# rehakvoj1/BIH-GPU-Raytracer

Hardware: NVIDIA B200
Metric: Mrays/s (higher is better)
Workload: dtype f32

## Files before the change

### bih-gpu-raytracer_b200/csrc/trace.cu

```cuda
#include "bihrt_internal.cuh"
#include <float.h>

#define FULL 0xffffffffu
#define NONE 0xFFFFFFFFu
#define TRACE_THREADS 128
#define TRACE_MIN_BLOCKS 8
constexpr int NODE_STEPS = 4;

#define OCT_MIXED 8
#define BOX_EPS 2.384185791015625e-07f

#define DET_EPS __uint_as_float(0x358637beu)

struct Hit { float t; int slot; };

__device__ __forceinline__ float fmin3(float a, float b, float c) { float r; asm("min.f32 %0, %1, %2, %3;" : "=f"(r) : "f"(a), "f"(b), "f"(c)); return r; }
__device__ __forceinline__ float fmax3(float a, float b, float c) { float r; asm("max.f32 %0, %1, %2, %3;" : "=f"(r) : "f"(a), "f"(b), "f"(c)); return r; }

__device__ __forceinline__ uint32_t pack_colour(uint32_t hits, int samples) {
    const float fh = (float)hits, fm = (float)(samples - (int)hits), fs = (float)samples;
    float cr = __fdiv_rn(__fadd_rn(__fmul_rn(fh, 255.f), __fmul_rn(fm, 20.f)), fs);
    float cb = __fdiv_rn(__fmul_rn(fm, 40.f), fs);
    cr = fmaxf(0.f, fminf(255.f, cr));
    cb = fmaxf(0.f, fminf(255.f, cb));
    return ((uint32_t)(int)cb << 16) | ((uint32_t)(int)cr << 8) | (uint32_t)(int)cr;
}

__device__ __forceinline__ float mt_det(float dx, float dy, float dz, float e1x, float e1y, float e1z, float e2x, float e2y, float e2z,
                                        float& px, float& py, float& pz) {
    px = __fsub_rn(__fmul_rn(dy, e2z), __fmul_rn(e2y, dz));
    py = __fsub_rn(__fmul_rn(dz, e2x), __fmul_rn(e2z, dx));
    pz = __fsub_rn(__fmul_rn(dx, e2y), __fmul_rn(e2x, dy));
    return __fadd_rn(__fadd_rn(__fmul_rn(e1x, px), __fmul_rn(e1y, py)), __fmul_rn(e1z, pz));
}
__device__ __forceinline__ float mt_u(float ox, float oy, float oz, const float4& q0, float px, float py, float pz, float inv,
                                      float& tx, float& ty, float& tz) {
    tx = __fsub_rn(ox, q0.x); ty = __fsub_rn(oy, q0.y); tz = __fsub_rn(oz, q0.z);
    return __fmul_rn(__fadd_rn(__fadd_rn(__fmul_rn(tx, px), __fmul_rn(ty, py)), __fmul_rn(tz, pz)), inv);
}
__device__ __forceinline__ float mt_v(float dx, float dy, float dz, float e1x, float e1y, float e1z, float tx, float ty, float tz, float inv,
                                      float& qx, float& qy, float& qz) {
    qx = __fsub_rn(__fmul_rn(ty, e1z), __fmul_rn(e1y, tz));
    qy = __fsub_rn(__fmul_rn(tz, e1x), __fmul_rn(e1z, tx));
    qz = __fsub_rn(__fmul_rn(tx, e1y), __fmul_rn(e1x, ty));
    return __fmul_rn(__fadd_rn(__fadd_rn(__fmul_rn(dx, qx), __fmul_rn(dy, qy)), __fmul_rn(dz, qz)), inv);
}

template <bool COUNTED, bool FIRST, bool RANGE = false, bool TWO_SIDED = false>
__device__ __forceinline__ void test_leaf(const char* __restrict__ first_tri, float ox, float oy, float oz,
                                          float dx, float dy, float dz, Hit& h, uint32_t& ntris, uint32_t& wleaf,
                                          const float* tlo_p = nullptr) {
    const float4* p = reinterpret_cast<const float4*>(first_tri);
    for (;;) {
        const float4 q0 = __ldg(p), q1 = __ldg(p + 1), q2 = __ldg(p + 2);
        if (COUNTED) { ntris++; const uint32_t am = __activemask(); wleaf += ((threadIdx.x & 31) == __ffs(am) - 1); }
        const float e1x = q0.w, e1y = q1.x, e1z = q1.y, e2x = q1.z, e2y = q1.w, e2z = q2.x;
        float px, py, pz;
        const float det = mt_det(dx, dy, dz, e1x, e1y, e1z, e2x, e2y, e2z, px, py, pz);
        if (!((TWO_SIDED ? fabsf(det) : det) < DET_EPS)) {
            const float inv = __frcp_rn(det);
            float tx, ty, tz;
            const float u = mt_u(ox, oy, oz, q0, px, py, pz, inv, tx, ty, tz);
            if (!(u < 0.f || u > 1.f)) {
                float qx, qy, qz;
                const float v = mt_v(dx, dy, dz, e1x, e1y, e1z, tx, ty, tz, inv, qx, qy, qz);
                if (!(v < 0.f || __fadd_rn(u, v) > 1.f)) {
                    const float t = __fmul_rn(__fadd_rn(__fadd_rn(__fmul_rn(e2x, qx), __fmul_rn(e2y, qy)), __fmul_rn(e2z, qz)), inv);
                    if (t > (RANGE ? *tlo_p : 0.f) && t < h.t) {
                        h.t = t; h.slot = (int)__float_as_uint(q2.w);
                        if (FIRST) break;
                    }
                }
            }
        }
        if (__float_as_uint(q2.z) & 1u) break;
        p += 3;
    }
}

template <int MODE, bool COUNTED, bool Q>
__global__ void __launch_bounds__(TRACE_THREADS, TRACE_MIN_BLOCKS) k_trace(TraceArgs a) {
    constexpr int STACK_DEPTH = Q ? STACK_DEPTH_QUALITY : STACK_DEPTH_PARITY;
    constexpr bool COVER = MODE == 1;
    constexpr bool OCTS = MODE == 1;
    constexpr bool LIST = MODE == 0 || MODE == 3 || MODE == 4;
    constexpr bool RANGE = MODE == 3 || MODE == 4;
    constexpr bool TWO_SIDED = MODE == 4;
    __shared__ __align__(16) float s_ray[TRACE_THREADS * 10];
    const int lane = threadIdx.x & 31;
    const uint32_t lt = (1u << lane) - 1u;
    float* my_ray = s_ray + threadIdx.x * 10;
    const char* __restrict__ nodes_b = reinterpret_cast<const char*>(a.nodes);
    const char* __restrict__ tris_b = reinterpret_cast<const char*>(a.tris);
    const BihTri* __restrict__ tris = a.tris;
    const uint32_t nu = a.hdr->nu;
    if (a.hdr->status != 0) return;
    if ((a.hdr->quality != 0) != Q) {
        if (blockIdx.x == 0 && threadIdx.x == 0 && a.status_map) *a.status_map = 0x100u;
        return;
    }
    const float blo[3] = { a.hdr->lo[0], a.hdr->lo[1], a.hdr->lo[2] }, bhi[3] = { a.hdr->hi[0], a.hdr->hi[1], a.hdr->hi[2] };
    uint32_t nnodes = 0, ntris = 0, maxsp = 0;
    uint32_t wnode = 0, wleaf = 0;

    uint64_t total;
    int tx = 1;
    if (LIST) total = a.tile_cost ? (((uint64_t)a.nrays + 1023u) >> 10) << 10 : (uint64_t)a.nrays;
    else {
        tx = (a.w + 31) / 32;
        const int ty = (a.h + 31) / 32, T = tx * ty;
        const int my_tiles = T > a.shard_index ? (T - a.shard_index + a.shard_count - 1) / a.shard_count : 0;
        total = ((uint64_t)my_tiles * 1024u) << a.gshift;
    }
    const int gshift = LIST ? 0 : a.gshift;
    const int nsamp = LIST ? 1 : ((a.s_end - a.s_begin) >> gshift);
    uint32_t my_queue = 0;
    if (a.queues > 1) { asm("mov.u32 %0, %%smid;" : "=r"(my_queue)); my_queue %= (uint32_t)a.queues; }
    uint64_t pool_next = 0, pool_end = 0;
    long long unit_t0 = 0; uint32_t unit_tile = 0xFFFFFFFFu;
    bool exhausted = false;

    uint64_t item = ~0ull;
    int s = 0, s0 = 0;
    uint32_t hits = 0, pixel = 0, pxy = 0;
    float ix = 1.f, iy = 1.f, iz = 1.f, nx = 0.f, ny = 0.f, nz = 0.f, bpad = 0.f;
    uint32_t cur = NONE;
    float rMin = 0.f, pMin = 0.f, pMax = 0.f;
    Hit h; h.t = FLT_MAX; h.slot = -1;
    bool tracing = false;
    uint4 stack[STACK_DEPTH];
    int sp = 0;
#define STACK_RESET() do { sp = 0; } while (0)
#define STACK_PUSH(item) do { stack[sp] = (item); sp++; } while (0)
#define STACK_POP(e) do { sp--; (e) = stack[sp]; } while (0)
    const uint32_t root_ref = BIH_REF_NODE(0, a.hdr->root_axis);
    const bool direct = MODE == 1 && gshift > 0 && !(a.flags & BIHRT_RENDER_COUNTS);
    const uint32_t ray_smem = (uint32_t)__cvta_generic_to_shared(my_ray);

    for (;;) {
        const uint32_t busy = ~__ballot_sync(FULL, cur == NONE);
        if (busy == 0) {
            bool want_item = false, finishing = false;
            if (cur == NONE) {
                if (tracing) {
                    tracing = false;
                    if (MODE == 1) hits += (h.slot >= 0);
                    else if (RANGE) {
                        const bool hit = h.slot >= 0;
                        const bool rec = a.out_u || a.out_v || a.out_ng;
                        float u = 0.f, v = 0.f, gx = 0.f, gy = 0.f, gz = 0.f;
                        int32_t prim = -1;
                        if (hit && (rec || a.out_prim)) {
                            const float4* tq = reinterpret_cast<const float4*>(tris + h.slot);
                            const float4 q0 = __ldg(tq), q1 = __ldg(tq + 1), q2 = __ldg(tq + 2);
                            prim = (int32_t)__float_as_uint(q2.y);
                            if (rec) {
                                const float e1x = q0.w, e1y = q1.x, e1z = q1.y, e2x = q1.z, e2y = q1.w, e2z = q2.x;
                                const float2 dxy = *reinterpret_cast<const float2*>(my_ray + 6);
                                const float dx = dxy.x, dy = dxy.y, dz = my_ray[8];
                                float px, py, pz, tx, ty, tz, qx, qy, qz;
                                const float inv = __frcp_rn(mt_det(dx, dy, dz, e1x, e1y, e1z, e2x, e2y, e2z, px, py, pz));
                                u = mt_u(my_ray[0], my_ray[2], my_ray[4], q0, px, py, pz, inv, tx, ty, tz);
                                v = mt_v(dx, dy, dz, e1x, e1y, e1z, tx, ty, tz, inv, qx, qy, qz);
                                gx = __fsub_rn(__fmul_rn(e1y, e2z), __fmul_rn(e1z, e2y));
                                gy = __fsub_rn(__fmul_rn(e1z, e2x), __fmul_rn(e1x, e2z));
                                gz = __fsub_rn(__fmul_rn(e1x, e2y), __fmul_rn(e1y, e2x));
                            }
                        }
                        if (a.out_t) a.out_t[item] = hit ? h.t : FLT_MAX;
                        if (a.out_slot) a.out_slot[item] = h.slot;
                        if (a.out_prim) a.out_prim[item] = prim;
                        if (a.out_u) a.out_u[item] = u;
                        if (a.out_v) a.out_v[item] = v;
                        if (a.out_ng) { float* g = a.out_ng + 3 * item; g[0] = gx; g[1] = gy; g[2] = gz; }
                    } else {
                        const uint64_t o = MODE == 0 ? item : (uint64_t)pixel * (uint32_t)a.spp + (uint32_t)(s0 + s);
                        if (a.out_t) a.out_t[o] = h.t;
                        if (a.out_slot) a.out_slot[o] = h.slot;
                        if (a.out_prim) a.out_prim[o] = h.slot >= 0 ? (int32_t)tris[h.slot].prim : -1;
                    }
                    s++;
                    if (s == nsamp) {
                        if (MODE == 1 && gshift > 0) finishing = true;
                        else if (MODE == 1 && (a.flags & BIHRT_RENDER_COUNTS)) a.fb[pixel] = hits;
                        else if (MODE == 1) a.fb[pixel] = pack_colour(hits, nsamp);
                        item = ~0ull;
                    }
                }
                want_item = (item == ~0ull);
            }
            if (MODE == 1 && gshift > 0) {
                const uint32_t fin = __ballot_sync(FULL, finishing);
                if (finishing) {
                    const uint32_t same = __match_any_sync(fin, pixel);
                    const uint32_t sum = __reduce_add_sync(same, hits);
                    if (lane == __ffs(same) - 1) {
                        if (direct) a.fb[pixel] = pack_colour(sum, nsamp << gshift);
                        else if (sum) atomicAdd(&a.fb[pixel], sum);
                    }
                }
            }
            if (!LIST && a.tile_cost && unit_tile != 0xFFFFFFFFu) {
                if (lane == 0) atomicMax(a.tile_cost + unit_tile, (uint32_t)min((unsigned long long)(clock64() - unit_t0) >> 8, 0xFFFFFFFFull));
                unit_tile = 0xFFFFFFFFu;
            }
            uint32_t want = __ballot_sync(FULL, want_item);
            while (want && !exhausted) {
                if (pool_next >= pool_end) {
                    uint64_t base = ~0ull;
                    uint32_t got = 0;
                    if (lane == 0) {
                        const uint32_t ilc = (uint32_t)a.il_count, ili = (uint32_t)a.il_index, ics = (uint32_t)a.il_cshift;
                        if (a.queues <= 1) {
                            const uint64_t fetched = atomicAdd(a.work, 32u); got = 32;
                            const uint64_t lu = fetched >> 5;
                            base = ilc > 1 ? ((((lu >> ics) * ilc + ili) << ics) | (lu & ((1u << ics) - 1u))) << 5 : fetched;
                            if (base >= total) base = ~0ull;
                        } else {
                            const uint32_t tshift = 10 + gshift, ushift = 5 + gshift;
                            const uint64_t ntile = (total + ((1ull << tshift) - 1)) >> tshift;
                            for (uint32_t k = 0; k < (uint32_t)a.queues; k++) {
                                uint32_t q = my_queue + k; if (q >= (uint32_t)a.queues) q -= (uint32_t)a.queues;
                                if (q >= ntile) continue;
                                const uint32_t upt = (1u << ushift) / ilc;
                                const uint64_t units = ((ntile - q + a.queues - 1) / a.queues) * upt;
                                if (ld_relaxed(a.work + q) >= units) continue;
                                const uint32_t u = atomicAdd(a.work + q, 1u);
                                if (u >= units) continue;
                                const uint32_t lu = u % upt;
                                const uint64_t b = (((uint64_t)(u / upt) * a.queues + q) << tshift) + ((uint64_t)((((lu >> ics) * ilc + ili) << ics) | (lu & ((1u << ics) - 1u))) << 5);
                                if (b < total) { base = b; got = 32; break; }
                            }
                        }
                    }
                    base = __shfl_sync(FULL, base, 0);
                    got = __shfl_sync(FULL, got, 0);
                    if (LIST && a.tile_cost && unit_tile != 0xFFFFFFFFu) {
                        if (lane == 0) atomicMax(a.tile_cost + unit_tile, (uint32_t)min((unsigned long long)(clock64() - unit_t0) >> 8, 0xFFFFFFFFull));
                        unit_tile = 0xFFFFFFFFu;
                    }
                    if (base == ~0ull) { exhausted = true; break; }
                    pool_next = base;
                    pool_end = min(base + got, total);
                    if (a.tile_cost && unit_tile == 0xFFFFFFFFu) {
                        const uint32_t m = (uint32_t)(base >> (10 + gshift));
                        unit_tile = a.tile_order ? __ldg(a.tile_order + m) : m;
                        unit_t0 = clock64();
                    }
                }
                const uint64_t avail = pool_end - pool_next;
                const uint32_t rank = __popc(want & lt);
                const bool served = want_item && (uint64_t)rank < avail;
                if (served) {
                    item = pool_next + rank; s = 0; hits = 0; want_item = false;
                    if (LIST && a.tile_cost) {
                        const uint32_t mi = (uint32_t)(item >> 10);
                        const uint64_t ray = ((uint64_t)(a.tile_order ? __ldg(a.tile_order + mi) : mi) << 10) | (item & 1023u);
                        item = ray < (uint64_t)a.nrays ? ray : ~0ull;
                        if (item == ~0ull) want_item = true;
                    }
                    if (MODE == 0 && a.perm && item != ~0ull) item = __ldg(a.perm + item);
                    if (!LIST) {
                        const uint64_t pix = item >> gshift;
                        s0 = a.s_begin + (int)((uint32_t)item & ((1u << gshift) - 1u)) * nsamp;
                        const uint32_t mi = (uint32_t)(pix >> 10), q = (uint32_t)pix & 1023u;
                        const uint32_t m = a.tile_order ? __ldg(a.tile_order + mi) : mi;
                        const int tile = a.shard_index + (int)m * a.shard_count;
                        const int px = (tile % tx) * 32 + (int)((q >> 5) & 3u) * 8 + (int)(q & 7u);
                        const int py = (tile / tx) * 32 + (int)(q >> 7) * 4 + (int)((q >> 3) & 3u);
                        if (px < a.w && py < a.h) { pixel = (uint32_t)(py * a.w + px); pxy = (uint32_t)px | ((uint32_t)py << 16); }
                        else item = ~0ull;
                        if (item == ~0ull) want_item = true;
                    }
                }
                pool_next += min((uint64_t)__popc(want), avail);
                want = __ballot_sync(FULL, want_item);
            }
            if (cur == NONE && item != ~0ull) {
                float ox, oy, oz, dx, dy, dz;
                float tlo = 0.f, thi = FLT_MAX;
                bool live = true;
                if (RANGE) {
                    const float4* p = reinterpret_cast<const float4*>(a.rays_iv + item);
                    const float4 r0 = __ldg(p), r1 = __ldg(p + 1);
                    ox = r0.x; oy = r0.y; oz = r0.z; dx = r1.x; dy = r1.y; dz = r1.z;
                    tlo = fmaxf(r0.w, 0.f);
                    live = r0.w == r0.w && tlo < r1.w;
                    thi = fminf(r1.w, FLT_MAX);
                } else if (MODE == 0) {
                    const float* p = reinterpret_cast<const float*>(a.rays + item);
                    ox = __ldg(p); oy = __ldg(p + 1); oz = __ldg(p + 2); dx = __ldg(p + 3); dy = __ldg(p + 4); dz = __ldg(p + 5);
                } else {
                    const int px = (int)(pxy & 0xFFFFu), py = (int)(pxy >> 16);
                    const float ru = (a.flags & BIHRT_RENDER_JITTER) ? bihrt_jitter(a.seed, pixel, (uint32_t)(s0 + s), 0) : 0.5f;
                    const float rv = (a.flags & BIHRT_RENDER_JITTER) ? bihrt_jitter(a.seed, pixel, (uint32_t)(s0 + s), 1) : 0.5f;
                    const float uu = __fdiv_rn(__fadd_rn((float)px, ru), (float)a.w);
                    const float vv = __fdiv_rn(__fadd_rn((float)py, rv), (float)a.h);
                    ox = a.cam.origin[0]; oy = a.cam.origin[1]; oz = a.cam.origin[2];
                    dx = __fsub_rn(__fadd_rn(__fadd_rn(a.cam.lower_left[0], __fmul_rn(uu, a.cam.horizontal[0])), __fmul_rn(vv, a.cam.vertical[0])), ox);
                    dy = __fsub_rn(__fadd_rn(__fadd_rn(a.cam.lower_left[1], __fmul_rn(uu, a.cam.horizontal[1])), __fmul_rn(vv, a.cam.vertical[1])), oy);
                    dz = __fsub_rn(__fadd_rn(__fadd_rn(a.cam.lower_left[2], __fmul_rn(uu, a.cam.horizontal[2])), __fmul_rn(vv, a.cam.vertical[2])), oz);
                }
                ix = __frcp_rn(dx); iy = __frcp_rn(dy); iz = __frcp_rn(dz);
                nx = -__fmul_rn(ox, ix); ny = -__fmul_rn(oy, iy); nz = -__fmul_rn(oz, iz);
                bpad = __fmul_rn(BOX_EPS, fmaxf(fmaxf(fabsf(nx) <= FLT_MAX ? fabsf(nx) : 0.f, fabsf(ny) <= FLT_MAX ? fabsf(ny) : 0.f),
                                                fabsf(nz) <= FLT_MAX ? fabsf(nz) : 0.f));
                *reinterpret_cast<float2*>(my_ray) = make_float2(ox, ix); *reinterpret_cast<float2*>(my_ray + 2) = make_float2(oy, iy);
                *reinterpret_cast<float2*>(my_ray + 4) = make_float2(oz, iz); *reinterpret_cast<float2*>(my_ray + 6) = make_float2(dx, dy);
                my_ray[8] = dz;
                if (RANGE) my_ray[9] = tlo;
                h.t = RANGE ? thi : (MODE == 0 && a.any_hit) ? a.tmax : FLT_MAX; h.slot = -1; STACK_RESET(); tracing = true;
                bool in = nu > 0 && live;
                float tMin = __fmul_rn(__fsub_rn(ix < 0.f ? bhi[0] : blo[0], ox), ix);
                float tMax = __fmul_rn(__fsub_rn(ix < 0.f ? blo[0] : bhi[0], ox), ix);
                const float tymin = __fmul_rn(__fsub_rn(iy < 0.f ? bhi[1] : blo[1], oy), iy);
                const float tymax = __fmul_rn(__fsub_rn(iy < 0.f ? blo[1] : bhi[1], oy), iy);
                if ((tMin > tymax) || (tymin > tMax)) in = false;
                if (tymin > tMin) tMin = tymin;
                if (tymax < tMax) tMax = tymax;
                const float tzmin = __fmul_rn(__fsub_rn(iz < 0.f ? bhi[2] : blo[2], oz), iz);
                const float tzmax = __fmul_rn(__fsub_rn(iz < 0.f ? blo[2] : bhi[2], oz), iz);
                if ((tMin > tzmax) || (tzmin > tMax)) in = false;
                if (tzmin > tMin) tMin = tzmin;
                if (tzmax < tMax) tMax = tzmax;
                if (in) {
                    const float tabs = fmaxf(fabsf(tMin), fabsf(tMax));
                    bpad = __fmaf_rn(BOX_EPS, tabs <= FLT_MAX ? tabs : FLT_MAX, bpad);
                    const float qnan = __uint_as_float(0x7fc00000u);
                    ix = fabsf(ix) <= FLT_MAX ? ix : qnan; iy = fabsf(iy) <= FLT_MAX ? iy : qnan; iz = fabsf(iz) <= FLT_MAX ? iz : qnan;
                    rMin = tMin; pMin = fmaxf(tMin, tlo); pMax = ((MODE == 0 && a.any_hit) || COVER || RANGE) ? fminf(tMax, h.t) : tMax;
                    if (nu == 1) { cur = BIH_REF_LEAFREF(0); pMin = -FLT_MAX; pMax = FLT_MAX; }
                    else if (pMin <= pMax) cur = root_ref;
                }
            }
            if (OCTS) {
                int oct = OCT_MIXED;
                if (gshift > 0) {
                    const bool w = cur != NONE;
                    const uint32_t xn = __ballot_sync(FULL, w && ix < 0.f), xp = __ballot_sync(FULL, w && ix > 0.f);
                    const uint32_t yn = __ballot_sync(FULL, w && iy < 0.f), yp = __ballot_sync(FULL, w && iy > 0.f);
                    const uint32_t zn = __ballot_sync(FULL, w && iz < 0.f), zp = __ballot_sync(FULL, w && iz > 0.f);
                    if (!((xn && xp) || (yn && yp) || (zn && zp))) oct = (xn != 0) | (yn != 0) << 1 | (zn != 0) << 2;
                }
                my_ray[9] = __int_as_float(oct);
            }
            if (__ballot_sync(FULL, cur != NONE || tracing) == 0 && exhausted &&
                __ballot_sync(FULL, item != ~0ull) == 0) break;
        }

#define BOX_SLAB(lx, ly, lz, hx, hy, hz, bn, bf)                                                            \
        do {                                                                                                \
            const float ax0 = __fmaf_rn((lx), ix, nx), ax1 = __fmaf_rn((hx), ix, nx);                       \
            const float ay0 = __fmaf_rn((ly), iy, ny), ay1 = __fmaf_rn((hy), iy, ny);                       \
            const float az0 = __fmaf_rn((lz), iz, nz), az1 = __fmaf_rn((hz), iz, nz);                       \
            float n_, f_;                                                                                   \
            if (OCT == OCT_MIXED) {                                                                         \
                n_ = fmaxf(fmaxf(fminf(ax0, ax1), fminf(ay0, ay1)), fminf(az0, az1));                       \
                f_ = fminf(fminf(fmaxf(ax0, ax1), fmaxf(ay0, ay1)), fmaxf(az0, az1));                       \
            } else {                                             \
                n_ = fmax3((OCT & 1) ? ax1 : ax0, (OCT & 2) ? ay1 : ay0, (OCT & 4) ? az1 : az0);            \
                f_ = fmin3((OCT & 1) ? ax0 : ax1, (OCT & 2) ? ay0 : ay1, (OCT & 4) ? az0 : az1);            \
            }                                                                                               \
            (bn) = __fsub_rn(n_, bpad);                                                                     \
            (bf) = __fadd_rn(f_, bpad);                                                                     \
        } while (0)
#define POP_VALID()                                                                                         \
        do {                                                                                                \
            cur = NONE;                                                                                     \
            if (COVER) {                                   \
                if (sp > 0) {                                                                               \
                    uint4 e;                                                                                \
                    STACK_POP(e);                                                                           \
                    cur = e.x; rMin = __uint_as_float(e.y); pMin = __uint_as_float(e.z); pMax = __uint_as_float(e.w); \
                }                                                                                           \
            } else while (sp > 0) {                                                                         \
                uint4 e;                                                                                    \
                STACK_POP(e);                                                                               \
                const float m = fminf(__uint_as_float(e.w), h.t);                                           \
                if (__uint_as_float(e.z) <= m) { cur = e.x; rMin = __uint_as_float(e.y); pMin = __uint_as_float(e.z); pMax = m; break; } \
            }                                                                                               \
        } while (0)
#ifdef BIHRT_DEBUG_STACK
#define DEBUG_STACK_TRAP() do { if (sp >= STACK_DEPTH) __trap(); } while (0)
#else
#define DEBUG_STACK_TRAP() do { } while (0)
#endif
#define NODE_PHASE(OCT_)                                                                                           \
        do {                                                                                                        \
            constexpr int OCT = (OCT_);                                                                             \
            for (;;) {                                                                                              \
                _Pragma("unroll (NODE_STEPS)")                                                                      \
                for (int rep = 0; rep < NODE_STEPS && (int)cur >= 0; rep++) {                                       \
                                    \
                    float2 oi;                                                                                      \
                    uint32_t ra;                                                                                    \
                    asm("mad.lo.u32 %0, %1, 8, %2;" : "=r"(ra) : "r"(cur & 3u), "r"(ray_smem));                     \
                    asm volatile("ld.shared.v2.f32 {%0, %1}, [%2];" : "=f"(oi.x), "=f"(oi.y) : "r"(ra));            \
                           \
                    const float4* np;                                                                               \
                    asm("mad.wide.u32 %0, %1, 64, %2;" : "=l"(np) : "r"(cur >> 2), "l"(nodes_b));                   \
                     \
                     \
                     \
                     \
                     \
                                                                          \
                    float4 nd, b0, b1, b2;                                                                          \
                    if (LIST) {                                                                                     \
                        asm("ld.global.nc.v8.f32 {%0,%1,%2,%3,%4,%5,%6,%7}, [%8];"                                  \
                            : "=f"(nd.x), "=f"(nd.y), "=f"(nd.z), "=f"(nd.w), "=f"(b0.x), "=f"(b0.y), "=f"(b0.z), "=f"(b0.w) : "l"(np)); \
                        asm("ld.global.nc.v8.f32 {%0,%1,%2,%3,%4,%5,%6,%7}, [%8];"                                  \
                            : "=f"(b1.x), "=f"(b1.y), "=f"(b1.z), "=f"(b1.w), "=f"(b2.x), "=f"(b2.y), "=f"(b2.z), "=f"(b2.w) : "l"(np + 2)); \
                    } else { nd = __ldg(np); b0 = __ldg(np + 1); b1 = __ldg(np + 2); b2 = __ldg(np + 3); }          \
                    if (COUNTED) { nnodes++; const uint32_t am = __activemask(); wnode += (lane == __ffs(am) - 1); } \
                    const uint32_t rl = __float_as_uint(nd.z), rr = __float_as_uint(nd.w);                          \
                    const bool neg = oi.y < 0.f;                                       \
                    const float t0 = __fmul_rn(__fsub_rn(nd.x, oi.x), oi.y);                          \
                    const float t1 = __fmul_rn(__fsub_rn(nd.y, oi.x), oi.y);                                        \
                    const float tn = neg ? t1 : t0, tf = neg ? t0 : t1;                                             \
                    const uint32_t refn = neg ? rr : rl, reff = neg ? rl : rr;                                      \
                     \
                     \
                     \
                     \
                                                              \
                    float bnL, bfL, bnR, bfR;                                                                       \
                    BOX_SLAB(b0.x, b0.y, b0.z, b0.w, b1.x, b1.y, bnL, bfL);                                         \
                    BOX_SLAB(b1.z, b1.w, b2.x, b2.y, b2.z, b2.w, bnR, bfR);                                         \
                     \
                    const float nLo = fmaxf(pMin, neg ? bnR : bnL), nHi = fmin3(pMax, tn, neg ? bfR : bfL);         \
                    const float fLo = fmax3(pMin, tf, neg ? bnL : bnR), fHi = fminf(pMax, neg ? bfL : bfR);         \
                    const bool go_near = (Q || rMin < tn) && (nLo <= nHi);    \
                    const bool go_far = (fLo <= fHi);                                                               \
                     \
                          \
                    if (go_near && go_far) {                                                                        \
                             \
                        if ((int)refn >= 0 && (int)reff < 0) {                                                      \
                            STACK_PUSH(make_uint4(refn, __float_as_uint(rMin), __float_as_uint(nLo), __float_as_uint(nHi))); \
                            cur = reff; rMin = tf; pMin = fLo; pMax = fHi;                                          \
                        } else {                                                                                    \
                            STACK_PUSH(make_uint4(reff, __float_as_uint(tf), __float_as_uint(fLo), __float_as_uint(fHi))); \
                            cur = refn; pMin = nLo; pMax = nHi;                                                     \
                        }                                                                                           \
                         \
                         \
                                                           \
                        if (COUNTED) { maxsp = max(maxsp, (uint32_t)sp); if (sp >= STACK_DEPTH) { maxsp = 0x7fffffffu; sp = STACK_DEPTH - 1; } } \
                        DEBUG_STACK_TRAP();                                                                         \
                    } else if (go_near) { cur = refn; pMin = nLo; pMax = nHi; }                                     \
                    else if (go_far) { cur = reff; rMin = tf; pMin = fLo; pMax = fHi; }                             \
                    else POP_VALID();                                                                               \
                }                                                                                                   \
                const uint32_t m_walk = __ballot_sync(FULL, (int)cur >= 0);                                         \
                if (m_walk == 0) break;                                                                             \
                const uint32_t m_wait = __ballot_sync(FULL, cur + 1u > 0x80000000u);   \
                if (__popc(m_wait) > __popc(m_walk)) break;                                                         \
            }                                                                                                       \
        } while (0)
        if constexpr (!OCTS) NODE_PHASE(OCT_MIXED);
        else switch (__float_as_int(my_ray[9])) {
            case 0: NODE_PHASE(0); break;
            case 1: NODE_PHASE(1); break;
            case 2: NODE_PHASE(2); break;
            case 3: NODE_PHASE(3); break;
            case 4: NODE_PHASE(4); break;
            case 5: NODE_PHASE(5); break;
            case 6: NODE_PHASE(6); break;
            case 7: NODE_PHASE(7); break;
            default: NODE_PHASE(OCT_MIXED); break;
        }
        if (cur + 1u > 0x80000000u) {
            const char* tp;
            asm("mad.wide.u32 %0, %1, 12, %2;" : "=l"(tp) : "r"(cur & 0x7FFFFFFCu), "l"(tris_b));
            const float2 dxy = *reinterpret_cast<const float2*>(my_ray + 6);
            test_leaf<COUNTED, COVER, RANGE, TWO_SIDED>(tp, my_ray[0], my_ray[2], my_ray[4], dxy.x, dxy.y, my_ray[8], h, ntris, wleaf, my_ray + 9);
            if (((LIST && a.any_hit) || COVER) && h.slot >= 0) { STACK_RESET(); cur = NONE; }
            else POP_VALID();
        }
#undef NODE_PHASE
#undef DEBUG_STACK_TRAP
#undef POP_VALID
#undef BOX_SLAB
#undef STACK_RESET
#undef STACK_PUSH
#undef STACK_POP
        __syncwarp();
    }

    if (COUNTED) {
#pragma unroll
        for (int o = 16; o > 0; o >>= 1) {
            nnodes += __shfl_xor_sync(FULL, nnodes, o);
            ntris += __shfl_xor_sync(FULL, ntris, o);
            maxsp = max(maxsp, __shfl_xor_sync(FULL, maxsp, o));
        }
        if (lane == 0) {
            atomicAdd(&a.counters[0], (unsigned long long)nnodes);
            atomicAdd(&a.counters[1], (unsigned long long)ntris);
            atomicMax(&a.counters[2], (unsigned long long)maxsp);
        }
        wnode = __reduce_add_sync(FULL, wnode); wleaf = __reduce_add_sync(FULL, wleaf);
        if (lane == 0) { atomicAdd(&a.counters[4], (unsigned long long)wnode); atomicAdd(&a.counters[5], (unsigned long long)wleaf); }
    }
}

__global__ void k_resolve(uint32_t* fb, int npix, int spp) {
    const int i = blockIdx.x * blockDim.x + threadIdx.x;
    if (i >= npix) return;
    fb[i] = pack_colour(fb[i], spp);
}

#define TILE_CLASSES 5
__device__ __forceinline__ int tile_class(uint32_t c, uint32_t mx) {
    int k = 0;
#pragma unroll
    for (int j = 1; j < TILE_CLASSES; j++) k += c < max(1u, mx >> j);
    return k;
}
__global__ void __launch_bounds__(1024) k_tile_order(uint32_t* __restrict__ cost, uint32_t* __restrict__ order, uint32_t ntiles) {
    __shared__ uint32_t s_w[TILE_CLASSES][32];
    __shared__ uint32_t s_max, s_base[TILE_CLASSES];
    const int lane = threadIdx.x & 31, w = threadIdx.x >> 5;
    const uint32_t per = (ntiles + 1023u) / 1024u, i0 = min(ntiles, threadIdx.x * per), i1 = min(ntiles, i0 + per);
    uint32_t mx = 0;
    for (uint32_t i = i0; i < i1; i++) mx = max(mx, cost[i]);
    mx = __reduce_max_sync(0xffffffffu, mx);
    if (lane == 0) s_w[0][w] = mx;
    __syncthreads();
    if (threadIdx.x == 0) { uint32_t m = 0; for (int k = 0; k < 32; k++) m = max(m, s_w[0][k]); s_max = m; }
    __syncthreads();
    mx = s_max;
    uint32_t cnt[TILE_CLASSES], inc[TILE_CLASSES];
#pragma unroll
    for (int k = 0; k < TILE_CLASSES; k++) cnt[k] = 0;
    for (uint32_t i = i0; i < i1; i++) {
        const int cl = tile_class(cost[i], mx);
#pragma unroll
        for (int k = 0; k < TILE_CLASSES; k++) cnt[k] += (cl == k);
    }
    __syncthreads();
#pragma unroll
    for (int k = 0; k < TILE_CLASSES; k++) {
        inc[k] = cnt[k];
#pragma unroll
        for (int o = 1; o < 32; o <<= 1) { const uint32_t t = __shfl_up_sync(0xffffffffu, inc[k], o); if (lane >= o) inc[k] += t; }
        if (lane == 31) s_w[k][w] = inc[k];
    }
    __syncthreads();
    if (threadIdx.x < TILE_CLASSES) {
        uint32_t run = 0;
        for (int j = 0; j < 32; j++) { const uint32_t x = s_w[threadIdx.x][j]; s_w[threadIdx.x][j] = run; run += x; }
        s_base[threadIdx.x] = run;
    }
    __syncthreads();
    if (threadIdx.x == 0) { uint32_t run = 0; for (int k = 0; k < TILE_CLASSES; k++) { const uint32_t x = s_base[k]; s_base[k] = run; run += x; } }
    __syncthreads();
    uint32_t pos[TILE_CLASSES];
#pragma unroll
    for (int k = 0; k < TILE_CLASSES; k++) pos[k] = s_base[k] + s_w[k][w] + inc[k] - cnt[k];
    for (uint32_t i = i0; i < i1; i++) {
        const int cl = tile_class(cost[i], mx);
#pragma unroll
        for (int k = 0; k < TILE_CLASSES; k++) if (cl == k) order[pos[k]++] = i;
    }
    __syncthreads();
    for (uint32_t i = i0; i < i1; i++) cost[i] = 0;
}

__global__ void __launch_bounds__(1024) k_tile_sort(uint32_t* __restrict__ cost, uint32_t* __restrict__ order, uint32_t ntiles) {
    __shared__ uint32_t s_cnt[256], s_off[256];
    if (threadIdx.x < 256) s_cnt[threadIdx.x] = 0;
    __syncthreads();
    for (uint32_t i = threadIdx.x; i < ntiles; i += 1024) atomicAdd(&s_cnt[min(255u, cost[i] >> 4)], 1u);
    __syncthreads();
    if (threadIdx.x == 0) { uint32_t run = 0; for (int b = 255; b >= 0; b--) { s_off[b] = run; run += s_cnt[b]; } }
    __syncthreads();
    for (uint32_t i = threadIdx.x; i < ntiles; i += 1024) order[atomicAdd(&s_off[min(255u, cost[i] >> 4)], 1u)] = i;
    __syncthreads();
    for (uint32_t i = threadIdx.x; i < ntiles; i += 1024) cost[i] = 0;
}

int bihrt_tile_order_launch(bihrt_ctx* c, uint32_t* cost, uint32_t* order, uint32_t ntiles, bool full_sort) {
    if (full_sort) k_tile_sort<<<1, 1024, 0, c->stream>>>(cost, order, ntiles);
    else k_tile_order<<<1, 1024, 0, c->stream>>>(cost, order, ntiles);
    c->kernel_launches += 1;
    BIHRT_CUDA(c, cudaGetLastError());
    return BIHRT_OK;
}

int bihrt_resolve_launch(bihrt_ctx* c, uint32_t* fb, int npix, int spp) {
    k_resolve<<<(npix + 255) / 256, 256, 0, c->stream>>>(fb, npix, spp);
    c->kernel_launches += 1;
    BIHRT_CUDA(c, cudaGetLastError());
    return BIHRT_OK;
}

template <int MODE, bool COUNTED, bool Q>
static int launch(bihrt_ctx* c, const TraceArgs& a) {
    int per_sm = c->opt_trace_blocks_per_sm;
    if (per_sm <= 0) {
        BIHRT_CUDA(c, cudaOccupancyMaxActiveBlocksPerMultiprocessor(&per_sm, k_trace<MODE, COUNTED, Q>, TRACE_THREADS, 0));
        if (per_sm < 1) per_sm = 1;
    }
    BIHRT_CUDA(c, cudaMemsetAsync(a.work, 0, 4 * 1024, c->stream));
    k_trace<MODE, COUNTED, Q><<<c->sm_count * per_sm, TRACE_THREADS, 0, c->stream>>>(a);
    c->kernel_launches += 1;
    BIHRT_CUDA(c, cudaGetLastError());
    return BIHRT_OK;
}

template <bool Q>
static int launch_mode(bihrt_ctx* c, const TraceArgs& a, int mode, bool counted) {
    switch (mode * 2 + (counted ? 1 : 0)) {
        case 0: return launch<0, false, Q>(c, a);
        case 1: return launch<0, true, Q>(c, a);
        case 2: return launch<1, false, Q>(c, a);
        case 3: return launch<1, true, Q>(c, a);
        case 4: return launch<2, false, Q>(c, a);
        case 5: return launch<2, true, Q>(c, a);
        case 6: return launch<3, false, Q>(c, a);
        case 8: return launch<4, false, Q>(c, a);
        default: return bihrt_fail(c, BIHRT_ERR_INVALID, "bad trace mode %d", mode);
    }
}

int bihrt_trace_launch(bihrt_ctx* c, const TraceArgs& a_in, int mode, bool counted) {
    TraceArgs a = a_in;
    const bool list = mode == 0 || mode == 3 || mode == 4;
    const int64_t rays = list ? a.nrays : (int64_t)a.w * a.h * (a.s_end - a.s_begin) / (a.shard_count > 0 ? a.shard_count : 1) / (a.il_count > 0 ? a.il_count : 1);
    const bool on = a.queues < 0 ? (rays >= (16ll << 20) && (list || a.gshift == 0)) : a.queues != 0;
    a.queues = on ? (c->sm_count < 1024 ? c->sm_count : 1024) : 1;
    uint32_t ntiles = 0;
    bihrt_ctx::TileKey key;
    if (!list) {
        const int tx = (a.w + 31) / 32, ty = (a.h + 31) / 32, T = tx * ty;
        const int mine = T > a.shard_index ? (T - a.shard_index + a.shard_count - 1) / a.shard_count : 0;
        if ((((uint64_t)mine * 1024u) << a.gshift) >= (1ull << 32) - (1ull << 24))
            return bihrt_fail(c, BIHRT_ERR_INVALID, "launch of %d tiles x 1024 pixels x %d lane groups exceeds the 32-bit work counter", mine, 1 << a.gshift);
    }
    const bool order_on = a.queues == 1 && (c->opt_tile_order > 1 || (c->opt_tile_order == 1 && rays >= (64ll << 10) && rays < (48ll << 20) && c->n >= 10000));
    if (order_on) {
        if (list) {
            if (a.nrays > 1024 && a.nrays <= (65536ll << 10)) { ntiles = (uint32_t)((a.nrays + 1023) >> 10); key.nrays = a.nrays; }
        } else {
            const int tx = (a.w + 31) / 32, ty = (a.h + 31) / 32, T = tx * ty;
            const int mine = T > a.shard_index ? (T - a.shard_index + a.shard_count - 1) / a.shard_count : 0;
            if (mine > 1 && mine <= 65536) ntiles = (uint32_t)mine;
            key.w = a.w; key.h = a.h; key.gshift = a.gshift; key.nsamp = a.s_end - a.s_begin; key.shard_index = a.shard_index;
            key.shard_count = a.shard_count; key.il_index = a.il_index; key.il_count = a.il_count; key.il_cshift = a.il_cshift;
        }
        key.mode = list ? mode : 1; key.ntiles = ntiles;
    }
    bihrt_ctx::TileSlot* slot = nullptr;
    if (ntiles) {
        for (auto& ts : c->tile_slots) if (ts.cap && ts.key == key) slot = &ts;
        if (!slot) {
            slot = &c->tile_slots[c->tile_next];
            c->tile_next = (c->tile_next + 1) % 4;
            slot->key = key; slot->valid = false;
        }
        if ((size_t)ntiles > slot->cap) {
            if (slot->cost) cudaFree(slot->cost);
            if (slot->order) cudaFree(slot->order);
            slot->cost = slot->order = nullptr; slot->cap = 0; slot->valid = false;
            if (cudaMalloc(&slot->cost, (size_t)ntiles * 4) != cudaSuccess || cudaMalloc(&slot->order, (size_t)ntiles * 4) != cudaSuccess) {
                cudaGetLastError();
                if (slot->cost) { cudaFree(slot->cost); slot->cost = nullptr; }
                slot = nullptr; ntiles = 0;
            } else slot->cap = ntiles;
        }
        if (slot) {
            if (!slot->valid) BIHRT_CUDA(c, cudaMemsetAsync(slot->cost, 0, (size_t)ntiles * 4, c->stream));
            a.tile_cost = slot->cost;
            a.tile_order = slot->valid ? slot->order : nullptr;
        }
    }
    a.status_map = c->d_status_map;
    int rc = c->built_quality ? launch_mode<true>(c, a, mode, counted) : launch_mode<false>(c, a, mode, counted);
    if (rc == BIHRT_OK && slot) {
        if ((rc = bihrt_tile_order_launch(c, slot->cost, slot->order, ntiles, rays < c->opt_tile_sort_below)) == BIHRT_OK) slot->valid = true;
    }
    return rc;
}
```

Baseline: 14690.

## Trim per-ray setup: colour table, camera-relative bounds, single-reduce octant, float tile divide

Several small setup costs in the trace kernel are cut. Each block precomputes a shared-memory colour table for small sample counts, so the per-pixel divides in pack_colour become a lookup. Scene bounds are pre-shifted by the camera origin in image modes, which drops a subtraction per slab. The six octant ballots become one __reduce_or_sync over a packed sign mask, and the tile divide/modulo is replaced by a float reciprocal with a one-step correction. These touch only per-ray or per-pixel setup rather than traversal, and they add a __syncthreads plus some shared memory per block.

```diff
diff --git a/bih-gpu-raytracer_b200/csrc/trace.cu b/bih-gpu-raytracer_b200/csrc/trace.cu
--- a/bih-gpu-raytracer_b200/csrc/trace.cu
+++ b/bih-gpu-raytracer_b200/csrc/trace.cu
@@ -8,6 +8,7 @@
 constexpr int NODE_STEPS = 4;
 
 #define OCT_MIXED 8
+#define COLOUR_TABLE_SAMPLES 64
 #define BOX_EPS 2.384185791015625e-07f
 
 #define DET_EPS __uint_as_float(0x358637beu)
@@ -87,6 +88,7 @@
     constexpr bool RANGE = MODE == 3 || MODE == 4;
     constexpr bool TWO_SIDED = MODE == 4;
     __shared__ __align__(16) float s_ray[TRACE_THREADS * 10];
+    __shared__ uint32_t s_colour[MODE == 1 ? COLOUR_TABLE_SAMPLES + 1 : 1];
     const int lane = threadIdx.x & 31;
     const uint32_t lt = (1u << lane) - 1u;
     float* my_ray = s_ray + threadIdx.x * 10;
@@ -99,7 +101,11 @@
         if (blockIdx.x == 0 && threadIdx.x == 0 && a.status_map) *a.status_map = 0x100u;
         return;
     }
-    const float blo[3] = { a.hdr->lo[0], a.hdr->lo[1], a.hdr->lo[2] }, bhi[3] = { a.hdr->hi[0], a.hdr->hi[1], a.hdr->hi[2] };
+    float blo[3] = { a.hdr->lo[0], a.hdr->lo[1], a.hdr->lo[2] }, bhi[3] = { a.hdr->hi[0], a.hdr->hi[1], a.hdr->hi[2] };
+    if (!LIST) {
+#pragma unroll
+        for (int k = 0; k < 3; k++) { blo[k] = __fsub_rn(blo[k], a.cam.origin[k]); bhi[k] = __fsub_rn(bhi[k], a.cam.origin[k]); }
+    }
     uint32_t nnodes = 0, ntris = 0, maxsp = 0;
     uint32_t wnode = 0, wleaf = 0;
 
@@ -135,6 +141,11 @@
 #define STACK_POP(e) do { sp--; (e) = stack[sp]; } while (0)
     const uint32_t root_ref = BIH_REF_NODE(0, a.hdr->root_axis);
     const bool direct = MODE == 1 && gshift > 0 && !(a.flags & BIHRT_RENDER_COUNTS);
+#define PIXEL_COLOUR(h) ((nsamp << gshift) <= COLOUR_TABLE_SAMPLES ? s_colour[(h)] : pack_colour((h), nsamp << gshift))
+    if (MODE == 1 && !(a.flags & BIHRT_RENDER_COUNTS) && (nsamp << gshift) <= COLOUR_TABLE_SAMPLES) {
+        for (int i = threadIdx.x; i <= (nsamp << gshift); i += TRACE_THREADS) s_colour[i] = pack_colour((uint32_t)i, nsamp << gshift);
+        __syncthreads();
+    }
     const uint32_t ray_smem = (uint32_t)__cvta_generic_to_shared(my_ray);
 
     for (;;) {
@@ -183,7 +194,7 @@
                     if (s == nsamp) {
                         if (MODE == 1 && gshift > 0) finishing = true;
                         else if (MODE == 1 && (a.flags & BIHRT_RENDER_COUNTS)) a.fb[pixel] = hits;
-                        else if (MODE == 1) a.fb[pixel] = pack_colour(hits, nsamp);
+                        else if (MODE == 1) a.fb[pixel] = PIXEL_COLOUR(hits);
                         item = ~0ull;
                     }
                 }
@@ -195,7 +206,7 @@
                     const uint32_t same = __match_any_sync(fin, pixel);
                     const uint32_t sum = __reduce_add_sync(same, hits);
                     if (lane == __ffs(same) - 1) {
-                        if (direct) a.fb[pixel] = pack_colour(sum, nsamp << gshift);
+                        if (direct) a.fb[pixel] = PIXEL_COLOUR(sum);
                         else if (sum) atomicAdd(&a.fb[pixel], sum);
                     }
                 }
@@ -266,8 +277,10 @@
                         const uint32_t mi = (uint32_t)(pix >> 10), q = (uint32_t)pix & 1023u;
                         const uint32_t m = a.tile_order ? __ldg(a.tile_order + mi) : mi;
                         const int tile = a.shard_index + (int)m * a.shard_count;
-                        const int px = (tile % tx) * 32 + (int)((q >> 5) & 3u) * 8 + (int)(q & 7u);
-                        const int py = (tile / tx) * 32 + (int)(q >> 7) * 4 + (int)((q >> 3) & 3u);
+                        int trow = __float2int_rz(__fmul_rn((float)tile, __fdividef(1.f, (float)tx))), tcol = tile - trow * tx;
+                        if (tcol >= tx) { trow++; tcol -= tx; }
+                        const int px = tcol * 32 + (int)((q >> 5) & 3u) * 8 + (int)(q & 7u);
+                        const int py = trow * 32 + (int)(q >> 7) * 4 + (int)((q >> 3) & 3u);
                         if (px < a.w && py < a.h) { pixel = (uint32_t)(py * a.w + px); pxy = (uint32_t)px | ((uint32_t)py << 16); }
                         else item = ~0ull;
                         if (item == ~0ull) want_item = true;
@@ -276,6 +289,7 @@
                 pool_next += min((uint64_t)__popc(want), avail);
                 want = __ballot_sync(FULL, want_item);
             }
+            uint32_t sg = 0;
             if (cur == NONE && item != ~0ull) {
                 float ox, oy, oz, dx, dy, dz;
                 float tlo = 0.f, thi = FLT_MAX;
@@ -311,15 +325,17 @@
                 if (RANGE) my_ray[9] = tlo;
                 h.t = RANGE ? thi : (MODE == 0 && a.any_hit) ? a.tmax : FLT_MAX; h.slot = -1; STACK_RESET(); tracing = true;
                 bool in = nu > 0 && live;
-                float tMin = __fmul_rn(__fsub_rn(ix < 0.f ? bhi[0] : blo[0], ox), ix);
-                float tMax = __fmul_rn(__fsub_rn(ix < 0.f ? blo[0] : bhi[0], ox), ix);
-                const float tymin = __fmul_rn(__fsub_rn(iy < 0.f ? bhi[1] : blo[1], oy), iy);
-                const float tymax = __fmul_rn(__fsub_rn(iy < 0.f ? blo[1] : bhi[1], oy), iy);
+#define SLAB_PLANE(b, o) (LIST ? __fsub_rn((b), (o)) : (b))
+                float tMin = __fmul_rn(SLAB_PLANE(ix < 0.f ? bhi[0] : blo[0], ox), ix);
+                float tMax = __fmul_rn(SLAB_PLANE(ix < 0.f ? blo[0] : bhi[0], ox), ix);
+                const float tymin = __fmul_rn(SLAB_PLANE(iy < 0.f ? bhi[1] : blo[1], oy), iy);
+                const float tymax = __fmul_rn(SLAB_PLANE(iy < 0.f ? blo[1] : bhi[1], oy), iy);
                 if ((tMin > tymax) || (tymin > tMax)) in = false;
                 if (tymin > tMin) tMin = tymin;
                 if (tymax < tMax) tMax = tymax;
-                const float tzmin = __fmul_rn(__fsub_rn(iz < 0.f ? bhi[2] : blo[2], oz), iz);
-                const float tzmax = __fmul_rn(__fsub_rn(iz < 0.f ? blo[2] : bhi[2], oz), iz);
+                const float tzmin = __fmul_rn(SLAB_PLANE(iz < 0.f ? bhi[2] : blo[2], oz), iz);
+                const float tzmax = __fmul_rn(SLAB_PLANE(iz < 0.f ? blo[2] : bhi[2], oz), iz);
+#undef SLAB_PLANE
                 if ((tMin > tzmax) || (tzmin > tMax)) in = false;
                 if (tzmin > tMin) tMin = tzmin;
                 if (tzmax < tMax) tMax = tzmax;
@@ -331,16 +347,15 @@
                     rMin = tMin; pMin = fmaxf(tMin, tlo); pMax = ((MODE == 0 && a.any_hit) || COVER || RANGE) ? fminf(tMax, h.t) : tMax;
                     if (nu == 1) { cur = BIH_REF_LEAFREF(0); pMin = -FLT_MAX; pMax = FLT_MAX; }
                     else if (pMin <= pMax) cur = root_ref;
+                    if (OCTS && cur != NONE) sg = (uint32_t)(ix < 0.f) | (uint32_t)(ix > 0.f) << 1 | (uint32_t)(iy < 0.f) << 2 |
+                                                  (uint32_t)(iy > 0.f) << 3 | (uint32_t)(iz < 0.f) << 4 | (uint32_t)(iz > 0.f) << 5;
                 }
             }
             if (OCTS) {
                 int oct = OCT_MIXED;
                 if (gshift > 0) {
-                    const bool w = cur != NONE;
-                    const uint32_t xn = __ballot_sync(FULL, w && ix < 0.f), xp = __ballot_sync(FULL, w && ix > 0.f);
-                    const uint32_t yn = __ballot_sync(FULL, w && iy < 0.f), yp = __ballot_sync(FULL, w && iy > 0.f);
-                    const uint32_t zn = __ballot_sync(FULL, w && iz < 0.f), zp = __ballot_sync(FULL, w && iz > 0.f);
-                    if (!((xn && xp) || (yn && yp) || (zn && zp))) oct = (xn != 0) | (yn != 0) << 1 | (zn != 0) << 2;
+                    const uint32_t any = __reduce_or_sync(FULL, sg);
+                    if (!(any & (any >> 1) & 0x15u)) oct = (any & 1u) | (any >> 1 & 2u) | (any >> 2 & 4u);
                 }
                 my_ray[9] = __int_as_float(oct);
             }
@@ -487,6 +502,7 @@
 #undef STACK_POP
         __syncwarp();
     }
+#undef PIXEL_COLOUR
 
     if (COUNTED) {
 #pragma unroll
```

After: 14920 (median of 6 runs). 1.02x the previous value.
